# gvanhorn38/multibox

Measured on AMD Instinct MI355X. Metric: images/sec (299x299, 5-AR priors) train, higher is better.
Workload: dtype bf16; 1 GPU; full train step: Inception-ResNet-v2 + multibox heads fwd, on-device matching+loss, bwd, RMSProp+EMA; 299x299, k=5 (P=646), BATCH_SIZE=64/GPU, MAX_NUM_BBOXES=13; global_batch=64, parallelism=dp1, hip_graph=True

## Files before the change

include/mbx.h:

```cpp
#ifndef MBX_H
#define MBX_H

#include <stddef.h>
#include <stdint.h>

#ifdef __cplusplus
extern "C" {
#endif

typedef void* mbx_stream_t;

typedef enum {
  MBX_OK = 0,
  MBX_ERR_INVALID_ARG = -1,
  MBX_ERR_UNSUPPORTED = -2,
  MBX_ERR_LAUNCH = -3,
  MBX_ERR_WORKSPACE = -4
} mbx_status;

int mbx_version(void);
const char* mbx_status_string(int status);

int mbx_priors_count(int k, const int* grids, int n_grids);

// ... 173 lines not shown
  const void* w; int32_t C_out, R, S;
  int32_t stride, transposed, pad_t, pad_l, H_out, W_out;
  void* y; int64_t y_img_stride; int32_t ldy;
  int32_t epilogue, relu, accumulate;
  const float* scale; const float* shift;
  const void* skip; int64_t skip_img_stride; int32_t ld_skip; float rscale;
  float* stats_partial;
  int32_t tile_config;
  const void* acc_src; int64_t acc_img_stride; int32_t ld_acc;
  int32_t* work_counter;
  int32_t max_workgroups;
  void* splitk_ws; int64_t splitk_ws_bytes;
  int32_t stats_rows_mod, stats_ld;
  const mbx_bn_bwd_stats* bn_bwd_stats;
  void* relu_bits; int32_t ld_bits;
  const mbx_bn_apply_desc* bn_apply;
  const mbx_bn_bwd_fused* bn_bwd;
} mbx_conv_desc;
#define MBX_CONV_TILE_CONFIGS 14
#define MBX_TILE_I5_BASE 32
#define MBX_TILE_I7 65
#define MBX_TILE_DIRECT3 96
#define MBX_TILE_DIRECTW 97
#define MBX_TILE_RESIDENT 98
#define MBX_TILE_PWRES 99
#define MBX_TILE_SPLITK_BASE 128
#define MBX_TILE_SPLITK_MAX 32

int mbx_conv_stats_rows(const mbx_conv_desc* desc );
int mbx_conv(const mbx_conv_desc* desc , mbx_stream_t stream);
int mbx_conv_supported(const mbx_conv_desc* desc );
int mbx_conv_pair(const mbx_conv_desc* a , const mbx_conv_desc* b , mbx_stream_t stream);
size_t mbx_conv_splitk_workspace_bytes(const mbx_conv_desc* desc );

int mbx_conv_wgrad(const mbx_conv_desc* desc , const void* dy,
                   int64_t dy_img_stride, int32_t ld_dy, float* dw, float* db, mbx_stream_t stream);

typedef struct {
  mbx_conv_desc desc;
  const void* dy; int64_t dy_img_stride; int32_t ld_dy;
  float scale;
  float* dw; float* db;
} mbx_wgrad_job;
typedef struct {
  int32_t n_layers, n_items;
  int64_t layers_off, items_off;
  int64_t queues_off, heads_off;
  double flops;
  int64_t tally_off;
} mbx_wgrad_plan_info;
#define MBX_WGRAD_DETERMINISTIC 1
#define MBX_WGRAD_SCATTER 2
size_t mbx_wgrad_plan_bytes(const mbx_wgrad_job* jobs , int n_jobs, int flags);
int mbx_wgrad_plan(const mbx_wgrad_job* jobs , int n_jobs, int flags, void* host_image, size_t bytes,
                   mbx_wgrad_plan_info* info );
int mbx_conv_wgrad_grouped(void* device_image , const mbx_wgrad_plan_info* info ,
                           mbx_stream_t stream);
int mbx_conv_wgrad_grouped_capped(void* device_image, const mbx_wgrad_plan_info* info , int max_workgroups,
                                  mbx_stream_t stream);

int mbx_conv_wgrad_scaled(const mbx_conv_desc* desc, const void* dy, int64_t dy_img_stride,
                          int32_t ld_dy, float scale, float* dw, float* db, mbx_stream_t stream);

int mbx_bn_finalize(const float* stats_partial , int rows, int C, int64_t count,
                    float eps, float decay, float* mean , float* rstd ,
                    float* moving_mean , float* moving_var ,
// ... 160 lines not shown
```

multibox_amd/_lib.py:

```python
from __future__ import annotations

import ctypes as C
import os

_HERE = os.path.dirname(os.path.abspath(__file__))
LIB_PATH = os.path.join(_HERE, "libmbx.so")

P = C.c_void_p
I = C.c_int
F = C.c_float
D = C.c_double
SZ = C.c_size_t


class PatchMeta(C.Structure):
    _fields_ = [("offset_y", C.c_int32), ("offset_x", C.c_int32), ("patch_h", C.c_int32), ("patch_w", C.c_int32),
                ("image_h", C.c_int32), ("image_w", C.c_int32), ("is_flipped", C.c_int32),
                ("max_to_keep", C.c_int32), ("restrictions", C.c_float * 4)]


_SIGS = {
    "mbx_version": (I, []),
    "mbx_status_string": (C.c_char_p, [I]),
    "mbx_priors_count": (I, [I, P, I]),
    "mbx_crc32c": (C.c_uint32, [P, C.c_uint64, C.c_uint32]),
    "mbx_generate_priors": (I, [P, I, D, D, I, P, I, P]),
    "mbx_decode_conf": (I, [P, P, P, I, I, F, P, P, P]),
    "mbx_match_workspace_bytes": (SZ, [I, I, I]),
    "mbx_match": (I, [P, P, P, P, F, I, I, I, P, P, P, SZ, P]),
    "mbx_match_extend": (I, [P, P, P, P, F, I, I, I, P, P, P]),
    "mbx_match_atss_supported": (I, [I, I, I, P, I]),
    "mbx_match_atss": (I, [P, P, I, P, P, P, I, I, I, I, P, P, P, P]),
    "mbx_loss_workspace_bytes": (SZ, [I]),
    "mbx_loss_fwd_bwd": (I, [P, P, I, P, P, F, F, I, I, I, P, P, P, P, SZ, P]),
    "mbx_loss_mined_workspace_bytes": (SZ, [I, I]),
    "mbx_loss_fwd_bwd_mined": (I, [P, P, I, P, P, F, F, I, I, I, P, P, P, I, I, P, P, SZ, P]),
    "mbx_loss_focal_workspace_bytes": (SZ, [I, I]),
    "mbx_loss_fwd_bwd_focal": (I, [P, P, I, P, P, F, F, I, I, I, P, P, P, F, F, F, I, I, P, P, SZ, P]),
    "mbx_loss_loc_workspace_bytes": (SZ, [I, I]),
    "mbx_loss_fwd_bwd_loc": (I, [P, P, I, P, P, F, F, I, I, I, P, P, P, I, F, F, F, F, I, I, P, P, SZ, P]),
    "mbx_decode_filter_topk": (I, [P, P, P, P, I, I, I, P, P, P, P, P]),
    "mbx_nms": (I, [P, P, P, P, I, I, C.c_double, P]),
    "mbx_merge_detections": (I, [P, P, P, P, I, I, I, C.c_double, P, P, P, P, P, P]),
    "mbx_merge_detections_voted": (I, [P, P, P, P, I, I, I, C.c_double, C.c_double, P, P, P, P, P, P, P]),
    "mbx_merge_detections_soft": (I, [P, P, P, P, I, I, I, I, C.c_double, C.c_double, C.c_double, C.c_double, P, P, P, P, P, P, P]),
    "mbx_coco_match": (I, [P, P, P, P, I, P, I, P, I, P, P, P, P, P]),
    "mbx_coco_accumulate_workspace": (SZ, [C.c_longlong, I, I, I]),
    "mbx_coco_accumulate": (I, [P, P, I, P, P, P, I, I, P, I, P, I, P, P, P, SZ, P]),
    "mbx_augment_workspace_bytes": (SZ, [I, I]),
    "mbx_augment_batch": (I, [P, P, I, I, I, P, P, P]),
    "mbx_extract_patches": (I, [P, P, I, I, P, P]),
    "mbx_conv_stats_rows": (I, [P]),
    "mbx_conv": (I, [P, P]),
    "mbx_conv_supported": (I, [P]),
    "mbx_conv_pair": (I, [P, P, P]),
    "mbx_conv_splitk_workspace_bytes": (SZ, [P]),
    "mbx_conv_wgrad": (I, [P, P, C.c_int64, I, P, P, P]),
    "mbx_conv_wgrad_scaled": (I, [P, P, C.c_int64, I, F, P, P, P]),
    "mbx_wgrad_plan_bytes": (SZ, [P, I, I]),
    "mbx_wgrad_plan": (I, [P, I, I, P, SZ, P]),
    "mbx_conv_wgrad_grouped": (I, [P, P, P]),
    "mbx_conv_wgrad_grouped_capped": (I, [P, P, I, P]),
    "mbx_bn_finalize": (I, [P, I, I, C.c_int64, F, F, P, P, P, P, P]),
    "mbx_bn_apply": (I, [P, C.c_int64, I, P, P, P, I, P, I, P]),
    "mbx_bn_moving_update": (I, [P, P, P, P, C.c_int64, F, P, P, P, P, F, P]),
    "mbx_bn_finalize_parts": (I, [P, P, P, I, C.c_int64, F, F, P, P, P, P, P]),
    "mbx_bn_apply_mapped": (I, [P, C.c_int64, I, P, P, P, I, P, I, P, P]),
    "mbx_bn_bwd_reduce_mapped": (I, [P, I, P, I, I, P, C.c_int64, I, P, P, P, P, P, P]),
    "mbx_bn_bwd_apply_mapped": (I, [P, I, P, I, I, P, C.c_int64, I, P, P, P, P, P, P, P]),
    "mbx_bn_apply_maxpool": (I, [P, I, I, I, I, P, P, P, I, P, C.c_int64, I, I, I, P, P]),
    "mbx_bn_bwd_rows_pooled": (I, [I, I, I, I]),
    "mbx_bn_bwd_reduce_pooled": (I, [P, C.c_int64, I, P, I, I, I, I, I, I, P, I, P, P, P, P, P]),
    "mbx_bn_bwd_apply_pooled": (I, [P, C.c_int64, I, P, I, I, I, I, I, I, P, I, P, P, P, P, P, P]),
    "mbx_bn_bwd_onepass_mapped": (I, [P, I, I, P, C.c_int64, I, P, P, P, P, P, P, I, P, P, P]),
    "mbx_bn_fold": (I, [P, P, P, F, I, P, P, P]),
    "mbx_bn_apply_fused": (I, [P, I, C.c_int64, F, F, P, C.c_int64, I, P, I, P, I, P, P, P, P, P]),
    "mbx_bn_apply_fused_mapped": (I, [P, I, C.c_int64, F, F, P, C.c_int64, I, P, I, P, I, P, P, P, P, P, P, P]),
    "mbx_bn_bwd_apply_rows": (I, [P, I, P, I, P, C.c_int64, I, P, P, P, P, P, P, P]),
    "mbx_bn_bwd_rows": (I, [C.c_int64, I]),
    "mbx_bn_bwd_onepass_workspace_bytes": (C.c_size_t, [I]),
    "mbx_bn_bwd_onepass_supported": (I, [C.c_int64, I, I]),
    "mbx_bn_bwd_onepass": (I, [P, I, I, P, C.c_int64, I, P, P, P, P, P, P, I, P, P]),
    "mbx_bn_bwd_reduce": (I, [P, I, P, I, I, P, C.c_int64, I, P, P, P, P, P]),
    "mbx_bn_bwd_finalize": (I, [P, I, I, C.c_int64, P, P, P]),
    "mbx_bn_bwd_apply": (I, [P, I, P, I, I, P, C.c_int64, I, P, P, P, P, P, P]),
    "mbx_maxpool_fwd": (I, [P, C.c_int64, I, I, I, I, I, I, I, P, C.c_int64, I, I, I, P, P]),
    "mbx_maxpool_bwd": (I, [P, C.c_int64, I, P, I, I, I, I, I, I, I, I, P, C.c_int64, I, I, P]),
    "mbx_avgpool_fwd": (I, [P, C.c_int64, I, I, I, I, I, I, I, P, C.c_int64, I, I, I, P]),
    "mbx_avgpool_bwd": (I, [P, C.c_int64, I, I, I, I, I, I, I, I, I, P, C.c_int64, I, I, P]),
# ... 69 lines not shown
```

multibox_amd/csrc/conv.hip:

```cpp
#include <stdlib.h>

#include "conv_common.h"

namespace {

template <int BM, int BN, int WNW, int WMW, int EV, int MODE = 0, int NSTG = 3>
__device__ __forceinline__ void conv_igemm3_body(const ConvK& p, const int bid_, const int nblk_) {
  constexpr bool SH = MODE == 2, PW = MODE == 1;
  static_assert(WNW * WMW == 4 || WNW * WMW == 8, "four or eight waves");
  constexpr int NT = 64 * WNW * WMW, RPP = NT / 8;
  constexpr int TN = BN / WNW, TM = BM / WMW, NI = TN / 16, MI = TM / 16;
  constexpr int PI = BM / RPP, WI = BN / RPP, NL = PI + WI;
  constexpr int STAGE = (BM + BN) * 8;
  extern __shared__ __attribute__((aligned(16))) u32x4 smem[];

  const int tid = threadIdx.x, lane = tid & 63;
  const int wave = wave_id();
  const int wn = wave % WNW, wm = wave / WNW;
  int lid = xcd_remap(bid_, nblk_);
  int split = 0;
  if constexpr (EV == 5) { const int nt = p.tiles_m * p.tiles_n; split = lid / nt; lid -= split * nt; }
  const int tile_n = lid % p.tiles_n, tile_m = lid / p.tiles_n;
  const int m0 = tile_m * BM, n0 = tile_n * BN;

  const __amdgpu_buffer_rsrc_t xr = make_rsrc(p.x, p.x_bytes);
  const __amdgpu_buffer_rsrc_t wr = make_rsrc(p.w, p.w_bytes);
  const int lrow = tid >> 3;
  const int chunk = (tid & 7) ^ (lrow & 7);
  const int chunkw = (tid & 7) ^ ((((lrow >> 3) & 3) << 1) | ((lrow >> 1) & 1));
  int hb[PI], wb[PI], ro[PI];
#pragma unroll
  for (int i = 0; i < PI; ++i) {
    const int m = m0 + lrow + RPP * i;
    const bool mv = m < p.M;
    const unsigned mm = mv ? (unsigned)m : 0u;
    int img, oh, ow;
    if (SH && p.parity) decode_pixel_parity(p, mm, img, oh, ow); else decode_pixel(p, mm, img, oh, ow);
    hb[i] = mv ? oh * p.mul - p.pad_t : -(1 << 24);
    wb[i] = ow * p.mul - p.pad_l;
    ro[i] = SH ? img * p.x_img_stride * 2 : (img * p.x_img_stride + (hb[i] * p.W_in + wb[i]) * p.ldx) * 2;
    if (PW && !mv) ro[i] = (int)kOOB;
  }
  int wo[WI];
#pragma unroll
  for (int i = 0; i < WI; ++i) {
    const int n = n0 + lrow + RPP * i;
    wo[i] = n < p.C_out ? n * p.Ktot * 2 : -1;
  }

  f32x4 acc[NI][MI];
#pragma unroll
  for (int a = 0; a < NI; ++a)
#pragma unroll
    for (int b = 0; b < MI; ++b) acc[a][b] = f32x4{0.f, 0.f, 0.f, 0.f};

  const int frow = lane & 15, fch = lane >> 4;
  const int fr0 = frow * 8 + (fch ^ (frow & 7));
  const int fr1 = frow * 8 + ((4 + fch) ^ (frow & 7));
  const int fwrow = 8 * (frow >> 2) + (frow & 3), fwkey = ((frow >> 2) << 1) | ((frow >> 1) & 1);
  const int fw0 = fwrow * 8 + (fch ^ fwkey);
  const int fw1 = fwrow * 8 + ((4 + fch) ^ fwkey);
  int kr0 = 0, ks0 = 0, kstep = 1, nk = (p.Ktot + 63) >> 6;
  if (SH && p.skip_taps) {
    const int mlast = min(m0 + BM, p.M) - 1;
    const int c0 = pixel_class(p, m0);
    if (c0 == pixel_class(p, mlast)) {
      kr0 = (p.pad_t + (c0 >> 1)) & 1;
      ks0 = (p.pad_l + (c0 & 1)) & 1;
      kstep = 2;
      nk = ((p.R - kr0 + 1) >> 1) * ((p.S - ks0 + 1) >> 1) * (p.C_in >> 6);
    }
  }
  int kt0 = 0;
  if constexpr (EV == 5) { kt0 = split * p.kps; nk = min(p.kps, nk - kt0); }
  int kc = chunk * 8 + kt0 * 64, kr = kr0, ks = ks0;
  while (kc >= p.C_in) { kc -= p.C_in; if ((ks += kstep) >= p.S) { ks = ks0; kr += kstep; } }
  const int ldx2 = p.ldx * 2;
  int st_issue = 0, st_comp = 0;
#define MBX_ISSUE_TILE(LT)                                                                                   \
  do {                                                                                                       \
    u32x4* sp = smem + st_issue * STAGE + wave * 64;                                                         \
    const bool kv = kr < p.R;                                                                                \
    if (PW) {                                                                                                \
      _Pragma("unroll") for (int i = 0; i < PI; ++i)                                                         \
        glds16(xr, sp + i * NT, (kv && ro[i] >= 0) ? (ro[i] + kc * 2) : (int)kOOB);                          \
    } else if (!SH) {                                                                                        \
      const int toff = (kr * p.W_in + ks) * ldx2 + kc * 2;                                                   \
      _Pragma("unroll") for (int i = 0; i < PI; ++i) {                                                       \
        const bool ok = kv && ((unsigned)(hb[i] + kr) < (unsigned)p.H_in) &&                                 \
                        ((unsigned)(wb[i] + ks) < (unsigned)p.W_in);                                         \
        glds16(xr, sp + i * NT, ok ? (ro[i] + toff) : (int)kOOB);                                            \
      }                                                                                                      \
    } else {                                                                                                 \
      _Pragma("unroll") for (int i = 0; i < PI; ++i) {                                                       \
        const int hn = hb[i] + kr, wn_ = wb[i] + ks;                                                         \
        const bool ok = kv && (((hn | wn_) & 1) == 0) && ((unsigned)(hn >> 1) < (unsigned)p.H_in) &&         \
                        ((unsigned)(wn_ >> 1) < (unsigned)p.W_in);                                           \
        glds16(xr, sp + i * NT, ok ? (ro[i] + ((hn >> 1) * p.W_in + (wn_ >> 1)) * ldx2 + kc * 2) : (int)kOOB); \
      }                                                                                                      \
    }                                                                                                        \
                                 \
    const int kb = (SH && kstep == 2) ? ((kr * p.S + ks) * p.C_in + kc + (chunkw - chunk) * 8) * 2                \
                                      : (((LT) + kt0) * 64 + chunkw * 8) * 2;                                  \
    const bool kvw = (SH && kstep == 2) ? kv : (kb < p.Ktot * 2);                                              \
    u32x4* sw = sp + BM * 8;                                                                                 \
    _Pragma("unroll") for (int i = 0; i < WI; ++i)                                                           \
      glds16(wr, sw + i * NT, (kvw && wo[i] >= 0) ? (wo[i] + kb) : (int)kOOB);                               \
    kc += 64;                                                                                                \
    while (kc >= p.C_in) { kc -= p.C_in; if ((ks += kstep) >= p.S) { ks = ks0; kr += kstep; } }              \
    st_issue = st_issue == NSTG - 1 ? 0 : st_issue + 1;                                                      \
  } while (0)

  static_assert(NSTG == 2 || NSTG == 3, "ring depth");
  u32x4* const probe_base = smem + (PI + WI - 1) * NT + wave * 64 + lane;
  MBX_ISSUE_TILE(0);
  if (NSTG == 3 && nk > 1) { MBX_ISSUE_TILE(1); wait_vmcnt<NL>(); } else wait_vmcnt<0>();
  lds_readback_wait(lds_readback_issue(probe_base));
  raw_barrier();
  for (int it = 0; it < nk; ++it) {
    const bool more = it + NSTG - 1 < nk;
    if (more) MBX_ISSUE_TILE(it + NSTG - 1);
    st_comp = st_comp == NSTG - 1 ? 0 : st_comp + 1;
    const int st_prev = st_comp == 0 ? NSTG - 1 : st_comp - 1;
#ifndef MBX_NO_PROBE_I3
    unsigned probe;
    if constexpr (NSTG == 3) {
      if (more) wait_vmcnt<NL>(); else wait_vmcnt<0>();
      probe = lds_readback_issue(probe_base + st_comp * STAGE);
    }
#endif
    {
      const u32x4* cP = smem + st_prev * STAGE + (wm * TM) * 8;
      const u32x4* cW = smem + st_prev * STAGE + BM * 8 + (wn * TN) * 8;
#pragma unroll
      for (int kk = 0; kk < 2; ++kk) {
        const int fr = kk ? fr1 : fr0, fw = kk ? fw1 : fw0;
        bf16x8 wf[NI], pf[MI];
#pragma unroll
        for (int a = 0; a < NI; ++a) wf[a] = __builtin_bit_cast(bf16x8, cW[(a >> 1) * 256 + (a & 1) * 32 + fw]);
#pragma unroll
        for (int b = 0; b < MI; ++b) pf[b] = __builtin_bit_cast(bf16x8, cP[b * 128 + fr]);
// ... 36 lines not shown
      }
    }
  } else {
    float s1[NA][8], s2[NA][8];
    conv_epilogue_direct<EV, SH, NI, MI, ((EV == 2 || EV == 6) && MI * NA >= 8 && MI % 2 == 0) ? 2 : MI>(p, acc, m0 + wm * TM + frow, n0 + cl0, s1, s2);
    if constexpr (EV == 1 || EV == 6) {
      float* red = reinterpret_cast<float*>(smem);
#pragma unroll
      for (int A = 0; A < NA; ++A) { row_sum16_x8(s1[A]); row_sum16_x8(s2[A]); }
#pragma unroll
      for (int A = 0; A < NA; ++A)
#pragma unroll
        for (int j = 0; j < 8; ++j) {
          const float x1 = s1[A][j], x2 = s2[A][j];
          if (frow == 0) {
            red[((wm * BN) + cl0 + 32 * A + j) * 2] = x1;
            red[((wm * BN) + cl0 + 32 * A + j) * 2 + 1] = x2;
          }
        }
      __syncthreads();
      if (tid < BN && n0 + tid < p.C_out) {
        float x1 = 0.f, x2 = 0.f;
#pragma unroll
        for (int w = 0; w < WMW; ++w) { x1 += red[(w * BN + tid) * 2]; x2 += red[(w * BN + tid) * 2 + 1]; }
        if constexpr (EV == 6) bw_stats_write(p, tile_m, n0 + tid, x1, x2); else stats_write(p, tile_m, n0 + tid, x1, x2);
      }
    }
  }
}

template <int BM, int BN, int WNW, int WMW, int EV, int MODE = 0, int NSTG = 3>
__global__ void __launch_bounds__(64 * WNW * WMW)
conv_igemm3_kernel(const ConvK p) {
  conv_igemm3_body<BM, BN, WNW, WMW, EV, MODE, NSTG>(p, (int)blockIdx.x, (int)gridDim.x);
}

template <int BM, int BN, int WNW, int WMW, int EV, int MODE = 0, int NSTG = 3>
__global__ void __launch_bounds__(64 * WNW * WMW)
conv_igemm3_pair_kernel(const ConvK p0, const ConvK p1, const int n0) {
  if ((int)blockIdx.x < n0) conv_igemm3_body<BM, BN, WNW, WMW, EV, MODE, NSTG>(p0, (int)blockIdx.x, n0);
  else conv_igemm3_body<BM, BN, WNW, WMW, EV, MODE, NSTG>(p1, (int)blockIdx.x - n0, (int)gridDim.x - n0);
}

constexpr int kSplitRows = 16;
__global__ void __launch_bounds__(256)
splitk_reduce_kernel(const float* __restrict__ part, int ksplit, long long slice_stride, int M, int C, int ldp,
                     unsigned short* __restrict__ y, int HW_out, long long y_img_stride, int ldy, float* __restrict__ stats,
                     int stats_mod, int stats_ld, float stats_cap) {
  __shared__ float red[kSplitRows][256][2];
  const int m0 = blockIdx.x * kSplitRows, tid = threadIdx.x;
  for (int cb = 0; cb < C; cb += 256) {
    const int cw = min(256, C - cb), c4 = (cw + 3) >> 2;
    if (cb) __syncthreads();
    for (int item = tid; item < kSplitRows * c4; item += 256) {
      const int r = item / c4, gq = item - r * c4, m = m0 + r, c = cb + 4 * gq;
      float4 a = make_float4(0.f, 0.f, 0.f, 0.f);
      if (m < M) {
        const float* src = part + (size_t)m * ldp + c;
        a = *reinterpret_cast<const float4*>(src);
        int sl = 1;
        for (; sl + 3 < ksplit; sl += 4) {
          const float4 b0 = *reinterpret_cast<const float4*>(src + (sl + 0) * slice_stride);
          const float4 b1 = *reinterpret_cast<const float4*>(src + (sl + 1) * slice_stride);
          const float4 b2 = *reinterpret_cast<const float4*>(src + (sl + 2) * slice_stride);
          const float4 b3 = *reinterpret_cast<const float4*>(src + (sl + 3) * slice_stride);
          a.x = (((a.x + b0.x) + b1.x) + b2.x) + b3.x; a.y = (((a.y + b0.y) + b1.y) + b2.y) + b3.y;
          a.z = (((a.z + b0.z) + b1.z) + b2.z) + b3.z; a.w = (((a.w + b0.w) + b1.w) + b2.w) + b3.w;
// ... 83 lines not shown
  static const int force = mbx_env_int("MBX_FORCE_CFG", -1);
  if (force >= 0) return force;
  if (desc_cfg > 0 && desc_cfg <= kNumCfgs) return desc_cfg - 1;
  {
    const long cols = (C_out + 127) / 128, tiles8 = ((M + 127) / 128) * cols;
    if (tiles8 >= 384 && (double)C_out >= 0.6 * (double)(cols * 128)) return 8;
  }
  if (C_out >= 256) {
    const long tiles5 = ((M + 255) / 256) * ((C_out + 127) / 128);
    const long rounds5 = (tiles5 + 255) / 256;
    if (tiles5 >= 128 && (double)tiles5 / (double)(rounds5 * 256) >= 0.7) return 5;
  }
  return pick_cfg(M, C_out);
}

struct PairCapture { ConvK k; int bm, bn, wnw, wmw, nstg, ev, mode, valid; };
thread_local PairCapture g_capture;

template <int BM, int BN, int WNW, int WMW, int EV, int NSTG>
int launch_pair_inst(const ConvK& a, const ConvK& b, hipStream_t s) {
  static bool attr = false;
  const size_t lds = NSTG * (size_t)(BM + BN) * 128;
  if (!attr) {
    (void)hipFuncSetAttribute(reinterpret_cast<const void*>(conv_igemm3_pair_kernel<BM, BN, WNW, WMW, EV, 0, NSTG>),
                              hipFuncAttributeMaxDynamicSharedMemorySize, (int)lds);
    attr = true;
  }
  const int n0 = a.tiles_m * a.tiles_n, n1 = b.tiles_m * b.tiles_n;
  hipLaunchKernelGGL((conv_igemm3_pair_kernel<BM, BN, WNW, WMW, EV, 0, NSTG>), dim3(n0 + n1), dim3(64 * WNW * WMW), lds, s, a, b, n0);
  MBX_LAUNCH_CHECK();
  return MBX_OK;
}

template <int BM, int BN, int WNW, int WMW, int NSTG = 3>
int launch_igemm(ConvK& k, hipStream_t s) {
  k.tiles_m = (k.M + BM - 1) / BM;
  k.tiles_n = (k.C_out + BN - 1) / BN;
  k.stats_cap = stats_cap_for(k.tiles_m);
  if (k.dry == 2) {
    g_capture.k = k; g_capture.bm = BM; g_capture.bn = BN; g_capture.wnw = WNW; g_capture.wmw = WMW; g_capture.nstg = NSTG;
    g_capture.ev = k.epi == MBX_EPI_STORE_F32 ? 5 : k.epi == MBX_EPI_RESIDUAL ? 4 : k.epi == MBX_EPI_AFFINE ? 3
                   : k.bw_n ? 6 : k.stats ? 1 : (k.accumulate || k.skip || k.bits) ? 2 : 0;
    g_capture.mode = k.shift ? 2 : k.pw ? 1 : 0;
    g_capture.valid = 1;
    return MBX_OK;
  }
  {
    const size_t lds = NSTG * (size_t)(BM + BN) * 128;
    const int ev = k.epi == MBX_EPI_STORE_F32 ? 5 : k.epi == MBX_EPI_RESIDUAL ? 4 : k.epi == MBX_EPI_AFFINE ? 3
                   : k.bw_n ? 6 : k.stats ? 1 : (k.accumulate || k.skip || k.bits) ? 2 : 0;
    static bool attr_set3[7] = {false, false, false, false, false, false, false};
#define MBX_LAUNCH_EV(EV)                                                                                     \
    case EV:                                                                                                  \
      if (!attr_set3[EV]) {                                                                                   \
        (void)hipFuncSetAttribute(reinterpret_cast<const void*>(conv_igemm3_kernel<BM, BN, WNW, WMW, EV, 0, NSTG>), \
                                  hipFuncAttributeMaxDynamicSharedMemorySize, (int)lds);                      \
        (void)hipFuncSetAttribute(reinterpret_cast<const void*>(conv_igemm3_kernel<BM, BN, WNW, WMW, EV, 1, NSTG>), \
                                  hipFuncAttributeMaxDynamicSharedMemorySize, (int)lds);                      \
        attr_set3[EV] = true;                                                                                 \
      }                                                                                                       \
      if (k.pw)                                                                                               \
        hipLaunchKernelGGL((conv_igemm3_kernel<BM, BN, WNW, WMW, EV, 1, NSTG>), dim3(k.tiles_m * k.tiles_n * (EV == 5 ? k.ksplit : 1)), \
                           dim3(64 * WNW * WMW), lds, s, k);                                                  \
      else                                                                                                    \
        hipLaunchKernelGGL((conv_igemm3_kernel<BM, BN, WNW, WMW, EV, 0, NSTG>), dim3(k.tiles_m * k.tiles_n * (EV == 5 ? k.ksplit : 1)), \
                           dim3(64 * WNW * WMW), lds, s, k);                                                  \
      break;
    static bool attr_sh[2] = {false, false};
#define MBX_LAUNCH_SH(EV, SLOT)                                                                               \
    do {                                                                                                      \
      if (!attr_sh[SLOT]) {                                                                                   \
        (void)hipFuncSetAttribute(reinterpret_cast<const void*>(conv_igemm3_kernel<BM, BN, WNW, WMW, EV, 2, NSTG>), \
                                  hipFuncAttributeMaxDynamicSharedMemorySize, (int)lds);                      \
        attr_sh[SLOT] = true;                                                                                 \
      }                                                                                                       \
      hipLaunchKernelGGL((conv_igemm3_kernel<BM, BN, WNW, WMW, EV, 2, NSTG>), dim3(k.tiles_m * k.tiles_n),      \
                         dim3(64 * WNW * WMW), lds, s, k);                                                    \
    } while (0)
    if (k.dry) return (k.shift && ev != 0 && ev != 2) ? MBX_ERR_UNSUPPORTED : MBX_OK;
    if (k.shift) {
      if (ev == 0) MBX_LAUNCH_SH(0, 0);
      else if (ev == 2) MBX_LAUNCH_SH(2, 1);
      else return MBX_ERR_UNSUPPORTED;
    } else
    switch (ev) {
      MBX_LAUNCH_EV(0) MBX_LAUNCH_EV(1) MBX_LAUNCH_EV(2) MBX_LAUNCH_EV(3) MBX_LAUNCH_EV(4) MBX_LAUNCH_EV(5) MBX_LAUNCH_EV(6)
    }
#undef MBX_LAUNCH_SH
#undef MBX_LAUNCH_EV
  }
  MBX_LAUNCH_CHECK();
  return MBX_OK;
}

}

extern "C" int mbx_conv_stats_rows(const mbx_conv_desc* d) {
  if (!d) return MBX_ERR_INVALID_ARG;
  if (d->stats_rows_mod > 0) return d->stats_rows_mod;
  const long M = (long)d->N * d->H_out * d->W_out;
  if (d->tile_config > kSplitFlag) return (int)((M + kSplitRows - 1) / kSplitRows);
  if (d->tile_config == kDirectCfg) return mbx_direct3_grid(d->N, d->H_out, d->W_out);
  if (d->tile_config == kDirectWCfg) { const int g = mbx_directw_grid(d->N, d->H_out, d->W_out); return g > 0 ? g : MBX_ERR_UNSUPPORTED; }
  if (d->tile_config == kResidentCfg) return mbx_resident_rows(d->N);
  if (d->tile_config == kI7Cfg) return (int)((M + 127) / 128);
  if (d->tile_config > kI5Flag) {
    const int i = d->tile_config - kI5Flag - 1;
    if (i >= mbx_i5_num_tiles) return MBX_ERR_INVALID_ARG;
    return (int)((M + mbx_i5_tiles[i][0] - 1) / mbx_i5_tiles[i][0]);
  }
  const TileCfg& c = kCfgs[choose_cfg(M, d->C_out, d->tile_config)];
  return (int)((M + c.BM - 1) / c.BM);
}

static int conv_impl(const mbx_conv_desc* d, mbx_stream_t stream, int dry);
extern "C" int mbx_conv(const mbx_conv_desc* d, mbx_stream_t stream) { return conv_impl(d, stream, 0); }
extern "C" int mbx_conv_supported(const mbx_conv_desc* d) { return conv_impl(d, nullptr, 1); }
extern "C" int mbx_conv_pair(const mbx_conv_desc* a, const mbx_conv_desc* b, mbx_stream_t stream) {
  PairCapture ca, cb;
  g_capture.valid = 0;
  int st = conv_impl(a, stream, 2);
  if (st != MBX_OK) return st;
  if (!g_capture.valid) return MBX_ERR_UNSUPPORTED;
  ca = g_capture;
  g_capture.valid = 0;
  st = conv_impl(b, stream, 2);
  if (st != MBX_OK) return st;
  if (!g_capture.valid) return MBX_ERR_UNSUPPORTED;
  cb = g_capture;
  if (ca.bm != cb.bm || ca.bn != cb.bn || ca.wnw != cb.wnw || ca.wmw != cb.wmw || ca.nstg != cb.nstg || ca.ev != cb.ev ||
      ca.mode != 0 || cb.mode != 0 || (ca.ev != 0 && ca.ev != 1 && ca.ev != 6) || ca.wnw != 2 || ca.wmw != 2 || ca.bn != 64)
    return MBX_ERR_UNSUPPORTED;
  ca.k.dry = cb.k.dry = 0;
  hipStream_t s = mbx_s(stream);
#define MBX_PAIR(BM_, NSTG_)                                                                                      \
  if (ca.bm == BM_ && ca.nstg == NSTG_)                                                                           \
    return ca.ev == 6 ? launch_pair_inst<BM_, 64, 2, 2, 6, NSTG_>(ca.k, cb.k, s)                                    \
           : ca.ev ? launch_pair_inst<BM_, 64, 2, 2, 1, NSTG_>(ca.k, cb.k, s) : launch_pair_inst<BM_, 64, 2, 2, 0, NSTG_>(ca.k, cb.k, s);
  MBX_PAIR(128, 2) MBX_PAIR(128, 3) MBX_PAIR(64, 2) MBX_PAIR(64, 3)
#undef MBX_PAIR
  return MBX_ERR_UNSUPPORTED;
}

extern "C" size_t mbx_conv_splitk_workspace_bytes(const mbx_conv_desc* d) {
  if (!d || d->tile_config <= kSplitFlag || d->tile_config > kSplitFlag + kSplitMax) return 0;
  int ksplit, kps;
  splitk_geom((d->R * d->S * d->C_in + 63) >> 6, d->tile_config - kSplitFlag, ksplit, kps);
  return (size_t)4 * d->N * d->H_out * d->W_out * (((d->C_out + 7) / 8) * 8) * ksplit;
}

static int conv_impl(const mbx_conv_desc* d, mbx_stream_t stream, int dry) {
  int st = check_desc(d);
  if (st != MBX_OK) return st;
  if (!d->w || !d->y) return MBX_ERR_INVALID_ARG;
  if ((reinterpret_cast<uintptr_t>(d->w) & 15)) return MBX_ERR_INVALID_ARG;
  const bool f32 = d->epilogue == MBX_EPI_STORE_F32;
  if (!f32 && (d->C_out % 8 || d->ldy % 8 || (reinterpret_cast<uintptr_t>(d->y) & 15))) return MBX_ERR_INVALID_ARG;
  if (d->epilogue == MBX_EPI_RESIDUAL && (!d->skip || d->ld_skip % 8 || (reinterpret_cast<uintptr_t>(d->skip) & 15)))
    return MBX_ERR_INVALID_ARG;
  if ((long long)d->N * d->y_img_stride >= (1LL << 31)) return MBX_ERR_UNSUPPORTED;
  if (d->stats_partial && (d->epilogue != MBX_EPI_STORE || d->accumulate || d->skip)) return MBX_ERR_INVALID_ARG;
  if (d->epilogue == MBX_EPI_STORE && d->skip && (d->ld_skip % 8 || (reinterpret_cast<uintptr_t>(d->skip) & 15))) return MBX_ERR_INVALID_ARG;
  MBX_ENTER();
  ConvK k;
  k.x = reinterpret_cast<const unsigned short*>(d->x);
  k.x_img_stride = (int)d->x_img_stride; k.ldx = d->ldx; k.H_in = d->H_in; k.W_in = d->W_in; k.C_in = d->C_in;
  k.w = reinterpret_cast<const unsigned short*>(d->w);
  k.C_out = d->C_out; k.R = d->R; k.S = d->S; k.Ktot = d->R * d->S * d->C_in;
  k.x_bytes = (unsigned)(2 * ((long long)(d->N - 1) * d->x_img_stride + ((long long)d->H_in * d->W_in - 1) * d->ldx + d->C_in));
  k.w_bytes = (unsigned)(2LL * d->C_out * k.Ktot);
  if (d->transposed) { k.mul = 1; k.shift = d->stride == 2 ? 1 : 0; } else { k.mul = d->stride; k.shift = 0; }
  k.pad_t = d->pad_t; k.pad_l = d->pad_l; k.W_out = d->W_out; k.HW_out = d->H_out * d->W_out;
  k.M = d->N * k.HW_out;
  k.y = d->y; k.y_img_stride = (int)d->y_img_stride; k.ldy = d->ldy;
// ... 86 lines not shown
  if (d->accumulate && d->acc_src) {
    if (d->ld_acc % 8 || (reinterpret_cast<uintptr_t>(d->acc_src) & 15) || (long long)d->N * d->acc_img_stride >= (1LL << 31))
      return MBX_ERR_INVALID_ARG;
    k.acc_src = reinterpret_cast<const unsigned short*>(d->acc_src); k.acc_img_stride = (int)d->acc_img_stride; k.ld_acc = d->ld_acc;
  } else {
    k.acc_src = reinterpret_cast<const unsigned short*>(d->y); k.acc_img_stride = (int)d->y_img_stride; k.ld_acc = d->ldy;
  }
  {
    const long long last_pix = (long long)k.HW_out - 1, span = ((d->C_out + 7) / 8) * 8;
    const long long yb = 2 * ((long long)(d->N - 1) * d->y_img_stride + last_pix * d->ldy + span);
    const long long sb = d->skip ? 2 * ((long long)(d->N - 1) * d->skip_img_stride + last_pix * d->ld_skip + span) : 0;
    const long long ab = 2 * ((long long)(d->N - 1) * k.acc_img_stride + last_pix * k.ld_acc + span);
    if (!f32 && (yb >= (1LL << 31) || sb >= (1LL << 31) || ab >= (1LL << 31))) return MBX_ERR_UNSUPPORTED;
    k.y_bytes = (unsigned)yb; k.skip_bytes = (unsigned)sb; k.acc_bytes = (unsigned)ab;
  }
  set_magic((unsigned)k.HW_out, k.mg_hw, k.sh_hw);
  set_magic((unsigned)k.W_out, k.mg_w, k.sh_w);
  k.pw = (d->R == 1 && d->S == 1 && d->pad_t == 0 && d->pad_l == 0 && d->stride == 1) ? 1 : 0;
  k.skip_taps = 0; k.parity = 0;
  k.work_counter = d->work_counter;
  k.max_wg = d->max_workgroups;
  k.dry = dry;
  k.ksplit = 1; k.kps = 1 << 30; k.y_split_stride = 0;
#ifdef MBX_I5_STAMPS
  {
    static const unsigned long long sp = getenv("MBX_I5_STAMP_PTR") ? strtoull(getenv("MBX_I5_STAMP_PTR"), nullptr, 10) : 0ull;
    k.stamps = reinterpret_cast<unsigned long long*>(sp);
    k.dbg = mbx_env_int("MBX_I5_DBG", 0);
    k.stagger = mbx_env_int("MBX_STAGGER", 0);
  }
#endif
  for (int c = 0; c < 4; ++c) { k.cls_m0[c] = 0; k.cls_hw[c] = 1; k.cls_w[c] = 1; }
  static const bool notap = mbx_env_char("MBX_NO_TAP_SKIP") == '1';
  if (k.shift && d->C_in % 64 == 0 && !notap) {
    int m0 = 0;
    for (int c = 0; c < 4; ++c) {
      const int hc = (d->H_out - (c >> 1) + 1) / 2, wc = (d->W_out - (c & 1) + 1) / 2;
      k.cls_m0[c] = m0;
      k.cls_hw[c] = hc * wc > 0 ? hc * wc : 1;
      k.cls_w[c] = wc > 0 ? wc : 1;
      m0 += d->N * hc * wc;
    }
    k.skip_taps = k.parity = 1;
  }
  if (k.bits && k.shift) return MBX_ERR_UNSUPPORTED;
  hipStream_t s = mbx_s(stream);
  if (d->tile_config > kSplitFlag) {
    const int S = d->tile_config - kSplitFlag;
    if (S < 2 || S > kSplitMax || d->transposed || d->bn_bwd_stats || d->relu_bits || d->epilogue != MBX_EPI_STORE || d->accumulate || d->skip || d->rscale != 0.f)
      return MBX_ERR_UNSUPPORTED;
    const int ldp = ((d->C_out + 7) / 8) * 8;
    int ksplit, kps;
    splitk_geom((k.Ktot + 63) >> 6, S, ksplit, kps);
    const long long slice = (long long)k.M * ldp;
    if (!d->splitk_ws || (reinterpret_cast<uintptr_t>(d->splitk_ws) & 15) || d->splitk_ws_bytes < (int64_t)(4 * slice * ksplit) ||
        slice * ksplit >= (1LL << 31))
      return MBX_ERR_WORKSPACE;
    ConvK g = k;
    g.epi = MBX_EPI_STORE_F32; g.stats = nullptr; g.relu = 0;
    g.y = d->splitk_ws; g.ldy = ldp; g.y_img_stride = k.HW_out * ldp;
    g.ksplit = ksplit; g.kps = kps; g.y_split_stride = slice;
    st = launch_igemm<128, 64, 2, 2>(g, s);
    if (st != MBX_OK || dry) return st;
    hipLaunchKernelGGL(splitk_reduce_kernel, dim3((k.M + kSplitRows - 1) / kSplitRows), dim3(256), 0, s, reinterpret_cast<const float*>(d->splitk_ws),
                       ksplit, slice, k.M, k.C_out, ldp, reinterpret_cast<unsigned short*>(k.y), k.HW_out,
                       (long long)k.y_img_stride, k.ldy, k.stats, k.stats_mod, k.stats_ld, stats_cap_for((k.M + kSplitRows - 1) / kSplitRows));
    MBX_LAUNCH_CHECK();
// ... 26 lines not shown
```

multibox_amd/csrc/conv_common.h:

```cpp
#pragma once
#include <type_traits>
#include "common.h"
#include "grid_barrier.h"

namespace mbx {

struct ConvK {
  const unsigned short* x; int x_img_stride, ldx, H_in, W_in, C_in;
  const unsigned short* w; int C_out, R, S, Ktot;
  unsigned x_bytes, w_bytes;
  unsigned y_bytes, skip_bytes, acc_bytes;
  int mul, shift, pad_t, pad_l, W_out, HW_out, M;
  void* y; int y_img_stride, ldy;
  int epi, relu, accumulate;
  const float* scale; const float* shiftv;
  const unsigned short* skip; int skip_img_stride, ld_skip; float rscale;
  const unsigned short* acc_src; int acc_img_stride, ld_acc;
  unsigned char* bits; int bits_ld; unsigned bits_bytes;
  float* stats;
  float stats_cap;
  int stats_mod, stats_ld;
  int bw_n, bw_mod;
  int bw_cb[4], bw_ldy[4], bw_sld[4];
  const unsigned short* bw_y[4];
// ... 167 lines not shown
  unsafeAtomicAdd(o, x1);
  unsafeAtomicAdd(o + 1, x2);
}
__device__ __forceinline__ void decode_pixel(const ConvK& p, unsigned m, int& img, int& oh, int& ow) {
  img = (int)fast_div(m, p.mg_hw, p.sh_hw);
  const int rem = (int)m - img * p.HW_out;
  oh = (int)fast_div((unsigned)rem, p.mg_w, p.sh_w);
  ow = rem - oh * p.W_out;
}
__device__ __forceinline__ void decode_pixel_parity(const ConvK& p, unsigned m, int& img, int& oh, int& ow) {
  const int c = ((int)m >= p.cls_m0[1]) + ((int)m >= p.cls_m0[2]) + ((int)m >= p.cls_m0[3]);
  const int m0 = c == 0 ? p.cls_m0[0] : c == 1 ? p.cls_m0[1] : c == 2 ? p.cls_m0[2] : p.cls_m0[3];
  const int hw = c == 0 ? p.cls_hw[0] : c == 1 ? p.cls_hw[1] : c == 2 ? p.cls_hw[2] : p.cls_hw[3];
  const int wc = c == 0 ? p.cls_w[0] : c == 1 ? p.cls_w[1] : c == 2 ? p.cls_w[2] : p.cls_w[3];
  unsigned r = m - (unsigned)m0;
  img = (int)(r / (unsigned)hw);
  r -= (unsigned)img * (unsigned)hw;
  const int a = (int)(r / (unsigned)wc), b = (int)r - a * wc;
  oh = 2 * a + (c >> 1);
  ow = 2 * b + (c & 1);
}
__device__ __forceinline__ int pixel_class(const ConvK& p, int m) {
  return (m >= p.cls_m0[1]) + (m >= p.cls_m0[2]) + (m >= p.cls_m0[3]);
}
constexpr unsigned kOOB = 0x80000000u;

__device__ __forceinline__ __amdgpu_buffer_rsrc_t make_rsrc(const void* p, unsigned bytes) {
  return __builtin_amdgcn_make_buffer_rsrc(const_cast<void*>(p), (short)0, (int)bytes, 0x00020000);
}
__device__ __forceinline__ u32x4 buf_load16(__amdgpu_buffer_rsrc_t r, unsigned byte_off) {
  return __builtin_amdgcn_raw_buffer_load_b128(r, (int)byte_off, 0, 0);
}

__device__ __forceinline__ int xcd_remap(int bid, int nblk) {
  const int xcd = bid & 7, q = nblk >> 3, r = nblk & 7;
  return (xcd < r ? xcd * (q + 1) : r * (q + 1) + (xcd - r) * q) + (bid >> 3);
}

__device__ __forceinline__ void glds16(__amdgpu_buffer_rsrc_t r, u32x4* lds_dst, int off) {
  __builtin_amdgcn_raw_ptr_buffer_load_lds(r, (__attribute__((address_space(3))) void*)lds_dst, 16, off, 0, 0, 0);
}
__device__ __forceinline__ int wave_id() { return __builtin_amdgcn_readfirstlane(threadIdx.x >> 6); }
__device__ __forceinline__ void raw_barrier() {
#ifndef MBX_UNFENCED_BARRIER
  asm volatile("" ::: "memory");
#endif
  __builtin_amdgcn_s_barrier();
#ifndef MBX_UNFENCED_BARRIER
  asm volatile("" ::: "memory");
#endif
}
__device__ __forceinline__ void lds_barrier() {
  asm volatile("s_waitcnt lgkmcnt(0)" ::: "memory");
  __builtin_amdgcn_s_barrier();
  asm volatile("" ::: "memory");
}

#ifdef MBX_NO_LANDING_PROBE
#define MBX_NO_PROBE_I3 1
#define MBX_NO_PROBE_I5 1
#define MBX_NO_PROBE_WG 1
#endif

template <int N>
__device__ __forceinline__ void wait_vmcnt() { asm volatile("s_waitcnt vmcnt(%0)" ::"n"(N) : "memory"); }

__device__ __forceinline__ unsigned lds_readback_issue(const void* lds_slot) {
// ... 247 lines not shown
```

Baseline: 4432 images/sec.

## Balance stride-2 conv tiles across XCDs by tap cost and extend tap-skip to C_in%32

Adds a host-computed block-to-tile deal for stride-2 parity-class convolutions. Tile rows are sorted by their tap count (the cost per tile) and dealt round-robin across XCD slots so that heavy and light classes spread evenly instead of sitting together on some XCDs. It also extends the tap-skipping stride-2 path to C_in divisible by 32 by masking the partial 64-channel chunk, and simplifies the k-walk for the skip case. It adds a debug export that reports the tile order, plus extra per-block index arithmetic in the kernel prologue.

```diff
diff --git a/include/mbx.h b/include/mbx.h
--- a/include/mbx.h
+++ b/include/mbx.h
@@ -229,6 +229,7 @@
 int mbx_conv_supported(const mbx_conv_desc* desc );
 int mbx_conv_pair(const mbx_conv_desc* a , const mbx_conv_desc* b , mbx_stream_t stream);
 size_t mbx_conv_splitk_workspace_bytes(const mbx_conv_desc* desc );
+int mbx_conv_stride2_order(const mbx_conv_desc* desc , int32_t* tile_of_block , int64_t capacity);
 
 int mbx_conv_wgrad(const mbx_conv_desc* desc , const void* dy,
                    int64_t dy_img_stride, int32_t ld_dy, float* dw, float* db, mbx_stream_t stream);
diff --git a/multibox_amd/_lib.py b/multibox_amd/_lib.py
--- a/multibox_amd/_lib.py
+++ b/multibox_amd/_lib.py
@@ -55,6 +55,7 @@
     "mbx_conv_supported": (I, [P]),
     "mbx_conv_pair": (I, [P, P, P]),
     "mbx_conv_splitk_workspace_bytes": (SZ, [P]),
+    "mbx_conv_stride2_order": (I, [P, P, C.c_int64]),
     "mbx_conv_wgrad": (I, [P, P, C.c_int64, I, P, P, P]),
     "mbx_conv_wgrad_scaled": (I, [P, P, C.c_int64, I, F, P, P, P]),
     "mbx_wgrad_plan_bytes": (SZ, [P, I, I]),
diff --git a/multibox_amd/csrc/conv.hip b/multibox_amd/csrc/conv.hip
--- a/multibox_amd/csrc/conv.hip
+++ b/multibox_amd/csrc/conv.hip
@@ -4,8 +4,33 @@
 
 namespace {
 
+struct S2Deal {
+  int row0[9];
+  int seg_end[7], seg_off[7];
+};
+__host__ __device__ __forceinline__ int stride2_tile(const int tiles_n, const S2Deal& d, const int bid, const int nblk) {
+  const int pos = xcd_remap(bid, nblk);
+  const int prow = pos / tiles_n, tn = pos - prow * tiles_n;
+  int x = 0, first = 0;
+#pragma unroll
+  for (int c = 1; c < 8; ++c)
+    if (prow >= d.row0[c]) { x = c; first = d.row0[c]; }
+  const int i = prow - first;
+  int j = 0;
+#pragma unroll
+  for (int c = 0; c < 8; ++c) {
+    const int n = d.row0[c + 1] - d.row0[c];
+    j += (n < i ? n : i) + ((c < x && n > i) ? 1 : 0);
+  }
+  int off = d.seg_off[0];
+#pragma unroll
+  for (int s = 1; s < 7; ++s)
+    if (j >= d.seg_end[s - 1]) off = d.seg_off[s];
+  return (j + off) * tiles_n + tn;
+}
+
 template <int BM, int BN, int WNW, int WMW, int EV, int MODE = 0, int NSTG = 3>
-__device__ __forceinline__ void conv_igemm3_body(const ConvK& p, const int bid_, const int nblk_) {
+__device__ __forceinline__ void conv_igemm3_body(const ConvK& p, const int bid_, const int nblk_, const S2Deal* deal = nullptr) {
   constexpr bool SH = MODE == 2, PW = MODE == 1;
   static_assert(WNW * WMW == 4 || WNW * WMW == 8, "four or eight waves");
   constexpr int NT = 64 * WNW * WMW, RPP = NT / 8;
@@ -18,6 +43,7 @@
   const int wave = wave_id();
   const int wn = wave % WNW, wm = wave / WNW;
   int lid = xcd_remap(bid_, nblk_);
+  if constexpr (SH) { if (p.parity) lid = stride2_tile(p.tiles_n, *deal, bid_, nblk_); }
   int split = 0;
   if constexpr (EV == 5) { const int nt = p.tiles_m * p.tiles_n; split = lid / nt; lid -= split * nt; }
   const int tile_n = lid % p.tiles_n, tile_m = lid / p.tiles_n;
@@ -68,13 +94,14 @@
       kr0 = (p.pad_t + (c0 >> 1)) & 1;
       ks0 = (p.pad_l + (c0 & 1)) & 1;
       kstep = 2;
-      nk = ((p.R - kr0 + 1) >> 1) * ((p.S - ks0 + 1) >> 1) * (p.C_in >> 6);
-    }
-  }
+      nk = ((p.R - kr0 + 1) >> 1) * ((p.S - ks0 + 1) >> 1) * ((p.C_in + 63) >> 6);
+    }
+  }
+  const bool skipw = SH && kstep == 2;
   int kt0 = 0;
   if constexpr (EV == 5) { kt0 = split * p.kps; nk = min(p.kps, nk - kt0); }
   int kc = chunk * 8 + kt0 * 64, kr = kr0, ks = ks0;
-  while (kc >= p.C_in) { kc -= p.C_in; if ((ks += kstep) >= p.S) { ks = ks0; kr += kstep; } }
+  if (!skipw) while (kc >= p.C_in) { kc -= p.C_in; if ((ks += kstep) >= p.S) { ks = ks0; kr += kstep; } }
   const int ldx2 = p.ldx * 2;
   int st_issue = 0, st_comp = 0;
 #define MBX_ISSUE_TILE(LT)                                                                                   \
@@ -95,18 +122,21 @@
       _Pragma("unroll") for (int i = 0; i < PI; ++i) {                                                       \
         const int hn = hb[i] + kr, wn_ = wb[i] + ks;                                                         \
         const bool ok = kv && (((hn | wn_) & 1) == 0) && ((unsigned)(hn >> 1) < (unsigned)p.H_in) &&         \
-                        ((unsigned)(wn_ >> 1) < (unsigned)p.W_in);                                           \
+                        ((unsigned)(wn_ >> 1) < (unsigned)p.W_in) && kc < p.C_in;                            \
         glds16(xr, sp + i * NT, ok ? (ro[i] + ((hn >> 1) * p.W_in + (wn_ >> 1)) * ldx2 + kc * 2) : (int)kOOB); \
       }                                                                                                      \
     }                                                                                                        \
-                                 \
-    const int kb = (SH && kstep == 2) ? ((kr * p.S + ks) * p.C_in + kc + (chunkw - chunk) * 8) * 2                \
-                                      : (((LT) + kt0) * 64 + chunkw * 8) * 2;                                  \
-    const bool kvw = (SH && kstep == 2) ? kv : (kb < p.Ktot * 2);                                              \
+     \
+    const int kcw = kc + (chunkw - chunk) * 8;                                                                 \
+    const int kb = skipw ? ((kr * p.S + ks) * p.C_in + kcw) * 2 : (((LT) + kt0) * 64 + chunkw * 8) * 2;        \
+    const bool kvw = skipw ? (kv && kcw < p.C_in) : (kb < p.Ktot * 2);                                         \
     u32x4* sw = sp + BM * 8;                                                                                 \
     _Pragma("unroll") for (int i = 0; i < WI; ++i)                                                           \
       glds16(wr, sw + i * NT, (kvw && wo[i] >= 0) ? (wo[i] + kb) : (int)kOOB);                               \
     kc += 64;                                                                                                \
+    if (skipw) {                             \
+      if (kc - chunk * 8 >= p.C_in) { kc = chunk * 8; if ((ks += 2) >= p.S) { ks = ks0; kr += 2; } }          \
+    } else                                                                                                   \
     while (kc >= p.C_in) { kc -= p.C_in; if ((ks += kstep) >= p.S) { ks = ks0; kr += kstep; } }              \
     st_issue = st_issue == NSTG - 1 ? 0 : st_issue + 1;                                                      \
   } while (0)
@@ -209,7 +239,14 @@
 template <int BM, int BN, int WNW, int WMW, int EV, int MODE = 0, int NSTG = 3>
 __global__ void __launch_bounds__(64 * WNW * WMW)
 conv_igemm3_kernel(const ConvK p) {
+  static_assert(MODE != 2, "the stride-2 walk is conv_igemm3_kernel_s2");
   conv_igemm3_body<BM, BN, WNW, WMW, EV, MODE, NSTG>(p, (int)blockIdx.x, (int)gridDim.x);
+}
+
+template <int BM, int BN, int WNW, int WMW, int EV, int NSTG = 3>
+__global__ void __launch_bounds__(64 * WNW * WMW)
+conv_igemm3_kernel_s2(const ConvK p, const S2Deal d) {
+  conv_igemm3_body<BM, BN, WNW, WMW, EV, 2, NSTG>(p, (int)blockIdx.x, (int)gridDim.x, &d);
 }
 
 template <int BM, int BN, int WNW, int WMW, int EV, int MODE = 0, int NSTG = 3>
@@ -359,6 +396,38 @@
   return MBX_OK;
 }
 
+void stride2_deal(const ConvK& k, const int BM, S2Deal& d) {
+  {
+    const int nblk = k.tiles_m * k.tiles_n, q = nblk >> 3, r = nblk & 7;
+    for (int x = 0; x < 8; ++x) d.row0[x] = (x * q + (x < r ? x : r) + k.tiles_n - 1) / k.tiles_n;
+    d.row0[8] = k.tiles_m;
+  }
+  struct Run { int t0, n, cost; } run[8];
+  int nr = 0, cur = 0;
+  for (int c = 0; c < 4 && k.parity; ++c) {
+    const int lo = k.cls_m0[c], hi = c < 3 ? k.cls_m0[c + 1] : k.M;
+    if (hi <= lo) continue;
+    const int first = (lo + BM - 1) / BM, end = hi == k.M ? k.tiles_m : hi / BM;
+    if (first > cur) { run[nr++] = Run{cur, first - cur, k.R * k.S + 1}; cur = first; }
+    if (end > cur) {
+      const int kr0 = (k.pad_t + (c >> 1)) & 1, ks0 = (k.pad_l + (c & 1)) & 1;
+      run[nr++] = Run{cur, end - cur, ((k.R - kr0 + 1) >> 1) * ((k.S - ks0 + 1) >> 1)};
+      cur = end;
+    }
+  }
+  if (cur < k.tiles_m) run[nr++] = Run{cur, k.tiles_m - cur, 0};
+  for (int a = 1; a < nr; ++a)
+    for (int b = a; b > 0 && run[b].cost > run[b - 1].cost; --b) { const Run t = run[b]; run[b] = run[b - 1]; run[b - 1] = t; }
+  int j = 0;
+  for (int s = 0; s < 7; ++s) {
+    if (s < nr) { d.seg_off[s] = run[s].t0 - j; j += run[s].n; d.seg_end[s] = j; }
+    else { d.seg_off[s] = 0; d.seg_end[s] = k.tiles_m; }
+  }
+}
+
+struct DealCapture { S2Deal d; int tiles_m, tiles_n, parity, valid; };
+thread_local DealCapture g_deal;
+
 template <int BM, int BN, int WNW, int WMW, int NSTG = 3>
 int launch_igemm(ConvK& k, hipStream_t s) {
   k.tiles_m = (k.M + BM - 1) / BM;
@@ -397,15 +466,21 @@
 #define MBX_LAUNCH_SH(EV, SLOT)                                                                               \
     do {                                                                                                      \
       if (!attr_sh[SLOT]) {                                                                                   \
-        (void)hipFuncSetAttribute(reinterpret_cast<const void*>(conv_igemm3_kernel<BM, BN, WNW, WMW, EV, 2, NSTG>), \
+        (void)hipFuncSetAttribute(reinterpret_cast<const void*>(conv_igemm3_kernel_s2<BM, BN, WNW, WMW, EV, NSTG>), \
                                   hipFuncAttributeMaxDynamicSharedMemorySize, (int)lds);                      \
         attr_sh[SLOT] = true;                                                                                 \
       }                                                                                                       \
-      hipLaunchKernelGGL((conv_igemm3_kernel<BM, BN, WNW, WMW, EV, 2, NSTG>), dim3(k.tiles_m * k.tiles_n),      \
-                         dim3(64 * WNW * WMW), lds, s, k);                                                    \
+      hipLaunchKernelGGL((conv_igemm3_kernel_s2<BM, BN, WNW, WMW, EV, NSTG>), dim3(k.tiles_m * k.tiles_n),      \
+                         dim3(64 * WNW * WMW), lds, s, k, deal);                                              \
     } while (0)
+    if (k.dry == 3 && k.shift && (ev == 0 || ev == 2)) {
+      stride2_deal(k, BM, g_deal.d);
+      g_deal.tiles_m = k.tiles_m; g_deal.tiles_n = k.tiles_n; g_deal.parity = k.parity; g_deal.valid = 1;
+    }
     if (k.dry) return (k.shift && ev != 0 && ev != 2) ? MBX_ERR_UNSUPPORTED : MBX_OK;
     if (k.shift) {
+      S2Deal deal;
+      stride2_deal(k, BM, deal);
       if (ev == 0) MBX_LAUNCH_SH(0, 0);
       else if (ev == 2) MBX_LAUNCH_SH(2, 1);
       else return MBX_ERR_UNSUPPORTED;
@@ -467,6 +542,18 @@
   MBX_PAIR(128, 2) MBX_PAIR(128, 3) MBX_PAIR(64, 2) MBX_PAIR(64, 3)
 #undef MBX_PAIR
   return MBX_ERR_UNSUPPORTED;
+}
+
+extern "C" int mbx_conv_stride2_order(const mbx_conv_desc* d, int32_t* tile_of_block, int64_t capacity) {
+  g_deal.valid = 0;
+  const int st = conv_impl(d, nullptr, 3);
+  if (st != MBX_OK) return st;
+  if (!g_deal.valid) return MBX_ERR_UNSUPPORTED;
+  const int nblk = g_deal.tiles_m * g_deal.tiles_n;
+  if (!tile_of_block || capacity < nblk) return MBX_ERR_INVALID_ARG;
+  for (int b = 0; b < nblk; ++b)
+    tile_of_block[b] = g_deal.parity ? stride2_tile(g_deal.tiles_n, g_deal.d, b, nblk) : xcd_remap(b, nblk);
+  return nblk;
 }
 
 extern "C" size_t mbx_conv_splitk_workspace_bytes(const mbx_conv_desc* d) {
@@ -619,7 +706,7 @@
 #endif
   for (int c = 0; c < 4; ++c) { k.cls_m0[c] = 0; k.cls_hw[c] = 1; k.cls_w[c] = 1; }
   static const bool notap = mbx_env_char("MBX_NO_TAP_SKIP") == '1';
-  if (k.shift && d->C_in % 64 == 0 && !notap) {
+  if (k.shift && d->C_in % 32 == 0 && !notap) {
     int m0 = 0;
     for (int c = 0; c < 4; ++c) {
       const int hc = (d->H_out - (c >> 1) + 1) / 2, wc = (d->W_out - (c & 1) + 1) / 2;
diff --git a/multibox_amd/csrc/conv_common.h b/multibox_amd/csrc/conv_common.h
--- a/multibox_amd/csrc/conv_common.h
+++ b/multibox_amd/csrc/conv_common.h
@@ -223,7 +223,7 @@
   return __builtin_amdgcn_raw_buffer_load_b128(r, (int)byte_off, 0, 0);
 }
 
-__device__ __forceinline__ int xcd_remap(int bid, int nblk) {
+__host__ __device__ __forceinline__ int xcd_remap(int bid, int nblk) {
   const int xcd = bid & 7, q = nblk >> 3, r = nblk & 7;
   return (xcd < r ? xcd * (q + 1) : r * (q + 1) + (xcd - r) * q) + (bid >> 3);
 }
```

Result: no change. 4463 images/sec (median of 6 runs) (+0.7%).
